# MarineRoboticsGroup/score

Measured on AMD Instinct MI355X. Metric: socp_iters_per_sec, higher is better.
Workload: dtype f64; 1 GPU; BASELINE configs[3]: manhattan RA-SLAM, 20 robots x 1000 poses, 4 beacons, SOCP relaxation, 1 trial(s)/GPU, ADMM loop alone (polish off) to eps 1e-07; n=146995, m=80979, nnz_P=946147, parallelism=independent x1

## Files before the change

score_amd/csrc/score_hip.hip:

```cpp
#include <hip/hip_runtime.h>
#include <sched.h>
#include <sys/prctl.h>
#include <time.h>
#include <hip/hip_ext.h>

#include <cstdio>
#include <cstring>
#include <malloc.h>
#include <mutex>
#include <string>
#include <memory>
#include <optional>
#include <vector>

#include "score_driver.hpp"
#include <future>
#include "score_assemble.hpp"
#include "score_gn_kernels.hpp"
#include "score_round.hpp"
#include "score_kernels.hpp"
#include "score_polish.hpp"
#include "score_polish_device.hpp"
#include "score_setup_device.hpp"
#include "score_prec_wave.hpp"
// ... 1840 lines not shown
            std::memset(h_rep, 0, total * sizeof(double));
            double* d_rep = nullptr;
            HIP_CHECK(hipHostGetDevicePointer((void**)&d_rep, h_rep, 0));
            rep.view(d_rep, total);
            rep_dres_off = n_pres;
            size_t o = 0;
            pres_part.view(d_rep + o, n_pres); h_pres = h_rep + o; o += n_pres;
            dres_part.view(d_rep + o, n_dres); h_dres = h_rep + o; o += n_dres;
            q_fpart.view(d_rep + o, n_fpart); h_newton = h_rep + o; o += n_fpart;
            q_gd.view(d_rep + o, n_gd); h_gd = h_rep + o; o += n_gd;
            h_meas = h_rep + o; d_meas = d_rep + o; o += n_meas;
            h_gate = (int32_t*)(h_rep + o); d_gate_host = (int32_t*)(d_rep + o); o += n_int;
            h_gate_live = (int32_t*)(h_rep + o); d_gate_live = (int32_t*)(d_rep + o); o += n_int;
            h_seq = (unsigned long long*)(h_rep + o); d_seq = (unsigned long long*)(d_rep + o);
            q_pcgdone.alloc(2 * (size_t)h.count);
            q_pcgdone.zero(stream);
            q_gate_used.view(q_pcgdone.d + h.count, h.count);
            ctl.alloc(2 * (size_t)h.count + (3 * (size_t)h.count + 1) / 2);
            q_step.view(ctl.d, h.count);
            q_gate_tol2.view(ctl.d + h.count, h.count);
            q_skip.view((int32_t*)(ctl.d + 2 * (size_t)h.count), h.count);
            q_reref.view((int32_t*)(ctl.d + 2 * (size_t)h.count) + h.count, h.count);
            q_fskip.view((int32_t*)(ctl.d + 2 * (size_t)h.count) + 2 * (size_t)h.count, h.count);
        }
        reset();
        pt.mark("reset");
        HIP_CHECK(sync_stream(stream));
        setup_tmp.release_all();
        for (auto& pb : setup_pinned) block_cache().give(pb.first, pb.second, st.device, true);
        setup_pinned.clear();
        pt.mark("staged uploads: drain");
    }

    void derive_rho_data(bool upload_penalties) {
        const HostSystem& h = *H;
        if (upload_penalties) {
            double* v = (double*)next_ring_slot(h.count * sizeof(double));
            for (int p = 0; p < h.count; ++p) v[p] = h.rho[p];
            fetch_words((int32_t*)rho.d, (const char*)v, 2 * h.count);
        }
        hipLaunchKernelGGL(k_kval, dim3(K.nblocks), dim3(kThreads), 0, stream, K.dev(), (const double*)K0d.d, (const double*)K1d.d,
                           (const double*)rho.d, K.val.d, (const int32_t*)nullptr);
        if (Kb.on) {
            const int64_t nnz = (int64_t)h.K.col.size();
            hipLaunchKernelGGL(k_band_pack, dim3((unsigned)((nnz + kThreads - 1) / kThreads)), dim3(kThreads), 0, stream, (const int32_t*)Kb.dst.d,
                               (const double*)K.val.d, Kb.V.d, nnz);
        }
        if (!h.factor_work.empty()) {
            FactorArgs fa{};
            fa.work = factor_work.d; fa.chains = chains.d; fa.levels = levels.d; fa.Hval = K.val.d;
            fa.pos_diag = kposd.d; fa.pos_sub = kposs.d; fa.fac = fac.d; fa.work_mat = q_work.d; fa.skip = nullptr;
            fa.diag_pos = kdiagpos.d; fa.dinv = dinv.d;
            launch_factor(fa, (int)h.factor_work.size(), false);
        }
        HIP_CHECK(hipGetLastError());
    }
    void join_init(const HostSystem& h) {
        n_join_items = (int)h.join_items.size(); n_join_chains = (int)h.join_chains.size(); n_join_seps = (int)h.join_sep_col.size();
        if (!n_join_items) return;
        for (const JoinChain& jc : h.join_chains)
            if (jc.n_seg - 1 > kJoinMaxSeps) throw std::runtime_error("internal: a segmented chain with more separators than the join kernel holds (build_system keeps such chains whole)");
        std::optional<UploadBatch> ub_join;
        ub_join.emplace();
        join_jc.upload(h.join_chains); join_items.upload(h.join_items);
        join_sep_col.upload(h.join_sep_col); join_sep_diag.upload(h.join_sep_diag);
        std::vector<int32_t> pc(2 * (size_t)n_join_seps), pp(2 * (size_t)n_join_seps);
// ... 613 lines not shown

    void launch_kp(const double* pdir, unsigned long long* ts = nullptr, int slot = -1) {
        SpmvArgs a = spmv_args(K, pdir);
        a.p = pdir; a.tstamp = ts;
        launch_spmv<MODE_KP>(K, a, slot);
    }
    void launch_kpb(const double* p_old, double* p_new, const double* rz_new, const double* rz_old,
                    unsigned long long* ts = nullptr, int slot = -1) {
        SpmvArgs a = spmv_args(K, p_old);
        a.tstamp = ts;
        a.p = p_old; a.z = z.d; a.p_out = p_new; a.rz_new = rz_new; a.rz_old = rz_old;
        launch_spmv<MODE_KPB>(K, a, slot);
    }

    void set_cg_iters(int k) {
        cg_iters = std::max(1, k);
        if (graph_exec) { (void)hipGraphExecDestroy(graph_exec); graph_exec = nullptr; }
    }

    void cg_reduction(std::vector<double>& out) {
        const HostSystem& h = *H;
        out.assign(h.count, 0.0);
        if (n_prec == 0) return;
        const double* a = h_meas;
        const double* b2 = h_meas + n_prec;
        for (int pi = 0; pi < h.count; ++pi) {
            double s0 = 0, s1 = 0;
            for (int i = active_part_ptr[pi]; i < active_part_ptr[pi + 1]; ++i) { s0 += a[i]; s1 += b2[i]; }
            out[pi] = s0 > 0 ? std::sqrt(std::max(0.0, s1) / s0) : 0.0;
        }
    }

    size_t ts_stride = 0;
    void enqueue_iteration(bool measure, bool first, unsigned long long* ts = nullptr) {
        auto slot = [&](int k) -> unsigned long long* { return ts ? ts + ts_stride * k : nullptr; };
        {
            SpmvArgs ra = spmv_args(G1, xtu.d);
            ra.tstamp = slot(0);
            ra.apply_update = first ? 0 : 1;
            ra.pfin = last_p;
            launch_spmv<MODE_RHS>(G1, ra, 0);
        }
        PrecArgs pa{};
        pa.work = prec_work.d; pa.chains = chains.d; pa.levels = levels.d; pa.rec = prec_rec.d; pa.fac = fac.d;
        pa.node_col = node_col.d; pa.diag_cols = diag_cols.d; pa.dinv = dinv.d; pa.done = done.d;
        pa.prec_part_ptr = prec_part_ptr.d; pa.kblk_part_ptr = kblk_part_ptr.d; pa.uni = uni_for(kblocks());
        pa.r = r.d; pa.r_in = r.d; pa.z = z.d; pa.p = p.d; pa.w = w.d; pa.xt = xtu.d; pa.kx = kx.d;
        pa.pw_part = pw_part.d;
        double* rz_cur = measure ? rz_meas0.d : rz_part0.d;
        double* p_cur = p.d;
        double* p_oth = p2.d;
        pa.p = p_cur; pa.rz_in = nullptr; pa.rz_out = rz_cur;
        pa.tstamp = slot(1);
        launch_prec<PREC_INIT>(pa, 1);
        launch_kp(p_cur, slot(2), 2);
        for (int j = 2; j <= cg_iters; ++j) {
            double* rz_nxt = (rz_cur == rz_part0.d) ? rz_part1.d : rz_part0.d;
            pa.p = p_cur; pa.rz_in = rz_cur; pa.rz_out = rz_nxt;
            pa.tstamp = (j == 2) ? slot(3) : nullptr;
            launch_prec<PREC_STEP>(pa, (j == 2) ? 3 : -1);
            launch_kpb(p_cur, p_oth, rz_nxt, rz_cur, (j == 2) ? slot(4) : nullptr, (j == 2) ? 4 : -1);
            std::swap(p_cur, p_oth);
            rz_cur = rz_nxt;
        }
        dbg_p = p_cur;
        ConeArgs ca = cone_args(xtu.d);
        if (measure) {
            pa.tstamp = nullptr;
            pa.p = p_cur; pa.rz_in = rz_cur; pa.rz_out = rz_meas1.d;
            launch_prec<PREC_STEP>(pa);
            VecArgs va{};
            va.first_row = vb_first.d; va.end_row = vb_end.d; va.blk_prob = vb_prob.d; va.done = done.d;
            va.prec_part_ptr = prec_part_ptr.d; va.kblk_part_ptr = kblk_part_ptr.d;
            va.pw_part = pw_part.d; va.p = p_cur; va.w = w.d; va.kx = kx.d; va.xt = xtu.d; va.x = xy.d;
            va.alpha_relax = st.alpha; va.rz_old = rz_cur; va.apply_alpha = 0;
            hipLaunchKernelGGL(k_xupdate, dim3(n_vblocks), dim3(kThreads), 0, stream, va);
        } else {
            ca.apply_alpha = 1; ca.pfin = p_cur; ca.rz_in = rz_cur;
            last_rz = rz_cur;
            last_p = p_cur;
        }
        ca.tstamp = slot(5);
        if (n_cone_blocks) {
            unsigned cgrid = (unsigned)n_cone_blocks;
            if (n_cone_blocks >= 16) { ca.xcd_chunk = (n_cone_blocks + 7) / 8; ca.n_blocks = n_cone_blocks; cgrid = 8u * (unsigned)ca.xcd_chunk; }
            launch_on_stream(k_cone, dim3(cgrid), dim3(kThreads), 0, 5, ca);
            ca.xcd_chunk = 0;
        }
        if (n_large_cones) {
            ca.tstamp = nullptr;
            hipLaunchKernelGGL(k_cone_wave, dim3((unsigned)((n_large_cones + 3) / 4)), dim3(kThreads), 0, stream, ca,
                               (const int2*)cone_large.d, n_large_cones);
        }
    }

    void time_iteration(int warmup, int iters, double* us, int with_events) {
        if (cg_iters != 2) throw std::runtime_error("score_time_iteration: needs cg_iters == 2");
        iters = std::max(1, iters);
        int khz = 0;
        HIP_CHECK(hipDeviceGetAttribute(&khz, hipDeviceAttributeWallClockRate, st.device));
        if (khz <= 0) throw std::runtime_error("score_time_iteration: no wall clock rate");
        for (int k = 0; k < 12; ++k) us[k] = 0.0;
        const int maxb = std::max(std::max(G1.nblocks, kblocks()) + 8, std::max(n_prec + n_help, n_cone_blocks + 8));
        ts_stride = (size_t)2 * maxb;
        const size_t per_iter = 6 * ts_stride, nslot = per_iter * iters;
        {
            std::vector<unsigned long long> hts(nslot);
            for (size_t i = 0; i < nslot; i += 2) { hts[i] = ~0ull; hts[i + 1] = 0ull; }
            DevBuf<unsigned long long> dts;
            dts.alloc(nslot);
            HIP_CHECK(hipMemcpyAsync(dts.d, hts.data(), nslot * sizeof(unsigned long long), hipMemcpyHostToDevice, stream));
            HIP_CHECK(sync_stream(stream));
            for (int i = 0; i < warmup; ++i) enqueue_iteration(false, i == 0);
            for (int i = 0; i < iters; ++i) enqueue_iteration(false, warmup == 0 && i == 0, dts.d + per_iter * i);
            HIP_CHECK(hipMemcpyAsync(hts.data(), dts.d, nslot * sizeof(unsigned long long), hipMemcpyDeviceToHost, stream));
            HIP_CHECK(sync_stream(stream));
            HIP_CHECK(hipGetLastError());
            for (int i = 0; i < iters; ++i)
                for (int k = 0; k < 6; ++k) {
                    const unsigned long long* p = &hts[per_iter * i + ts_stride * k];
                    unsigned long long t0 = ~0ull, t1 = 0ull;
                    for (int b = 0; b < maxb; ++b) { t0 = std::min(t0, p[2 * b]); t1 = std::max(t1, p[2 * b + 1]); }
                    if (t1 > t0) us[k] += (double)(t1 - t0) * 1e3 / (double)khz / iters;
                }
            if (trace_on("stamps")) {
                const unsigned long long* base = &hts[per_iter * (size_t)(iters - 1)];
                unsigned long long t00 = ~0ull;
                for (size_t j = 0; j < per_iter; j += 2) t00 = std::min(t00, base[j]);
                for (int k = 0; k < 6; ++k)
                    for (int b = 0; b < maxb; ++b) {
                        const unsigned long long a0 = base[ts_stride * k + 2 * (size_t)b], a1 = base[ts_stride * k + 2 * (size_t)b + 1];
                        if (a0 == ~0ull || a1 == 0ull) continue;
                        std::printf("STAMP %d %d %.3f %.3f\n", k, b, (double)(a0 - t00) * 1e3 / (double)khz, (double)(a1 - t00) * 1e3 / (double)khz);
                    }
            }
        }
        if (!with_events) return;
        std::vector<hipEvent_t> evs((size_t)12 * iters, nullptr);
        struct EvFree {
            std::vector<hipEvent_t>& v;
            ~EvFree() { for (hipEvent_t e : v) if (e) (void)hipEventDestroy(e); }
        } ev_free{evs};
        for (auto& e : evs) HIP_CHECK(hipEventCreate(&e));
        for (int i = 0; i < warmup; ++i) enqueue_iteration(false, false);
        for (int i = 0; i < iters; ++i) {
            tev = evs.data() + (size_t)12 * i;
            enqueue_iteration(false, false);
// ... 158 lines not shown
                               (const double*)Dd.d, (const double*)Ed.d, ob, n, m);
            try {
                copy_out({{x, {ob, (size_t)n}}, {y, {ob + n, (size_t)m}}, {s_out, {ob + n + m, (size_t)m}}});
            } catch (...) {
                block_cache().give(ob, got, st.device, false);
                throw;
            }
            block_cache().give(ob, got, st.device, false);
            return;
        }
        std::vector<double> hx((size_t)(n + m)), hs((size_t)m);
        copy_out({{hx.data(), {xy.d, hx.size()}}, {m ? hs.data() : nullptr, {s.d, hs.size()}}});
        if (x) for (int64_t i = 0; i < n; ++i) x[i] = hx[i] * h.D[i];
        if (y) for (int64_t i = 0; i < m; ++i) y[i] = hx[n + i] * h.E[i];
        if (s_out) for (int64_t i = 0; i < m; ++i) s_out[i] = hs[i] / h.E[i];
    }

    int64_t get_vec(const char* name, double* out, int64_t len) {
        const HostSystem& h = *H;
        const double* src = nullptr;
        int64_t sz = 0;
        bool host = false;
        std::string nm(name);
        if (nm == "xt") { src = xtu.d; sz = h.n_tot; }
        else if (nm == "u") { src = xtu.d + h.n_tot; sz = h.m_tot; }
        else if (nm == "x") { src = xy.d; sz = h.n_tot; }
        else if (nm == "y") { src = xy.d + h.n_tot; sz = h.m_tot; }
        else if (nm == "s") { src = s.d; sz = h.m_tot; }
        else if (nm == "r") { src = r.d; sz = h.n_tot; }
        else if (nm == "z") { src = z.d; sz = h.n_tot; }
        else if (nm == "p") { src = dbg_p ? dbg_p : ((cg_iters % 2 == 1) ? p.d : p2.d); sz = h.n_tot; }
        else if (nm == "w") { src = w.d; sz = h.n_tot; }
        else if (nm == "kx") { src = kx.d; sz = h.n_tot; }
        else if (nm == "D" && h.device_setup) { src = Dd.d; sz = h.n_tot; }
        else if (nm == "E" && h.device_setup) { src = Ed.d; sz = h.m_tot; }
        else if (nm == "D") { src = h.D.data(); sz = h.n_tot; host = true; }
        else if (nm == "E") { src = h.E.data(); sz = h.m_tot; host = true; }
        else if (nm == "K0" || nm == "K1" || nm == "Aval" || nm == "G1val" || nm == "G2val" || nm == "qs" || nm == "bs" || nm == "invD" || nm == "invE") {
            const int64_t nk = (int64_t)h.K.col.size(), na = (int64_t)h.A.ptr[(size_t)h.m_tot];
            const int64_t n1 = h.device_setup ? g1_nnz : (int64_t)h.G1.col.size(), n2 = (int64_t)h.G2.ptr[(size_t)h.n_tot];
            if (nm == "K0") { src = K0d.d; sz = nk; } else if (nm == "K1") { src = K1d.d; sz = nk; }
            else if (nm == "Aval") { src = A_val.d; sz = na; } else if (nm == "G1val") { src = G1.val.d; sz = n1; }
            else if (nm == "G2val") { src = G2.val.d; sz = n2; } else if (nm == "qs") { src = q.d; sz = h.n_tot; }
            else if (nm == "bs") { src = b.d; sz = h.m_tot; } else if (nm == "invD") { src = invD.d; sz = h.n_tot; }
            else { src = invE.d; sz = h.m_tot; }
        }
        else if (nm == "Acol" || nm == "Aptr" || nm == "G1col" || nm == "G1ptr" || nm == "G2col" || nm == "G2ptr" || nm == "G2split" || nm == "Kcol_dev" || nm == "Kptr_dev") {
            const int64_t nk = (int64_t)h.K.col.size(), na = (int64_t)h.A.ptr[(size_t)h.m_tot];
            const int64_t n1 = h.device_setup ? g1_nnz : (int64_t)h.G1.col.size(), n2 = (int64_t)h.G2.ptr[(size_t)h.n_tot];
            const int32_t* isrc = nullptr;
            if (nm == "Acol") { isrc = A_col.d; sz = na; } else if (nm == "Aptr") { isrc = A_ptr.d; sz = h.m_tot + 1; }
            else if (nm == "G1col") { isrc = G1.col.d; sz = n1; } else if (nm == "G1ptr") { isrc = G1.ptr.d; sz = h.n_tot + 1; }
            else if (nm == "G2col") { isrc = G2.col.d; sz = n2; } else if (nm == "G2ptr") { isrc = G2.ptr.d; sz = h.n_tot + 1; }
            else if (nm == "G2split") { isrc = G2.split.d; sz = h.n_tot; } else if (nm == "Kcol_dev") { isrc = K.col.d; sz = nk; }
            else { isrc = K.ptr.d; sz = h.n_tot + 1; }
            if (out && len > 0) {
                std::vector<int32_t> tmp((size_t)std::min(len, sz));
                HIP_CHECK(sync_stream(stream));
                staged_d2h(tmp.data(), isrc, tmp.size() * sizeof(int32_t), stream);
                HIP_CHECK(sync_stream(stream));
                for (size_t i = 0; i < tmp.size(); ++i) out[i] = (double)tmp[i];
            }
            return sz;
        }
        else if (nm == "setup_scalars") {
            sz = 5 * (int64_t)h.count;
// ... 5 lines not shown
            return sz;
        }
        else if (nm == "device_setup") {
            if (out && len > 0) out[0] = h.device_setup ? 1.0 : 0.0;
            return 1;
        }
        else if (nm == "Kval") { src = K.val.d; sz = (int64_t)h.K.col.size(); }
        else if (nm == "rep") {
            const double v[3] = {(double)h.rep, (double)h.K.col.size(), (double)(h.device_setup ? (size_t)g1_nnz : h.G1.col.size())};
            if (out && len > 0) std::memcpy(out, v, sizeof(double) * (size_t)std::min<int64_t>(len, 3));
            return 3;
        }
        else if (nm == "links") {
            double v[6] = {(double)link_plan.pairs_total, (double)link_plan.pairs_used, (double)n_link_u, (double)n_link_items, (double)link_rounds, 0.0};
            if (n_link_probs && out) {
                std::vector<int32_t> stt((size_t)n_link_probs);
                HIP_CHECK(sync_stream(stream));
                for (int set = 0; set < 2; ++set) {
                    if (!link_set_on[set]) continue;
                    HIP_CHECK(hipMemcpy(stt.data(), link_status[set].d, sizeof(int32_t) * (size_t)n_link_probs, hipMemcpyDeviceToHost));
                    for (int32_t x : stt) v[5] += x;
                }
            }
            if (out && len > 0) std::memcpy(out, v, sizeof(double) * (size_t)std::min<int64_t>(len, 6));
            return 6;
        }
        else if (nm == "link_pairs") {
            const std::vector<int32_t>& pc = link_plan.pair_cols;
            const int64_t np_ = n_link_items ? (int64_t)pc.size() : 0;
            if (out) for (int64_t i = 0; i < np_ && i < len; ++i) out[i] = (double)pc[(size_t)i];
            return np_;
        }
        else if (nm == "fac") { src = fac.d; sz = (int64_t)h.fac_doubles; }
        else if (nm == "newton_probe_arm") {
            if (!Q.available) return -1;
            if (out && len > 0) {
                for (hipEvent_t e : np_ev) (void)hipEventDestroy(e);
                np_ev.assign((size_t)2 * kProbeCap, nullptr);
                for (auto& e : np_ev)
                    if (hipEventCreate(&e) != hipSuccess) return -2;
                np_slots.clear();
                np_armed = true;
                out[0] = 1.0;
            }
            return 1;
        }
        else if ((nm == "ag_device_check" || nm == "polish_build_check") && h.device_setup) return -1;
        else if (nm == "ag_device_check") {
            if (out && len >= 7) {
                auto down_i = [&](const int32_t* d, size_t cnt) {
                    std::vector<int32_t> v(cnt);
                    if (cnt) staged_d2h(v.data(), d, cnt * sizeof(int32_t), stream);
                    HIP_CHECK(sync_stream(stream));
                    return v;
                };
                auto down_d = [&](const double* d, size_t cnt) {
                    std::vector<double> v(cnt);
                    if (cnt) staged_d2h(v.data(), d, cnt * sizeof(double), stream);
                    HIP_CHECK(sync_stream(stream));
                    return v;
                };
                auto mism = [](const std::vector<int32_t>& x, const std::vector<int32_t>& y) {
                    double c = 0;
                    for (size_t i = 0; i < y.size(); ++i) c += x[i] != y[i];
                    return c;
                };
// ... 1911 lines not shown
```

score_amd/csrc/score_host.hpp:

```cpp
#pragma once

#include <algorithm>
#include <atomic>
#include <cmath>
#include <chrono>
#include <cstdint>
#include <cstdio>
#include <cstring>
#include <numeric>
#include <stdexcept>
#include <string>
#include <thread>
#include <condition_variable>
#include <functional>
#include <mutex>

#include <pthread.h>
#include <sched.h>
#include <sys/resource.h>
#include <vector>

#include "../../include/score_hip.h"

namespace score {
// ... 547 lines not shown
}

inline void chain_level_layout(int bs, int radix, int N0, std::vector<ChainLevelDesc>& levels, size_t& fac_size,
                               int& scratch_nodes) {
    const int b2 = bs * bs;
    int N = N0, vec_off = 0, lds_off = 0;
    size_t off = 0;
    levels.clear();
    for (int lvl = 0;; ++lvl) {
        ChainLevelDesc L{};
        L.N = N;
        L.vec_off = (lvl == 0) ? -1 : vec_off;
        if (lvl > 0) vec_off += N;
        const bool last = (N <= radix - 1);
        L.p = last ? 0 : radix;
        L.inv_p = last ? 0u : ((1u << 20) / (uint32_t)radix + 1u);
        L.lds_off = lds_off;
        lds_off += N * bs + (last ? 0 : N / radix) + 1;
        const int nsep = last ? 0 : N / radix;
        L.nsep = nsep;
        L.nruns = nsep + 1;
        L.P = last ? N : radix - 1;
        L.offR = (int64_t)off; off += (size_t)2 * b2 * L.P * L.nruns;
        L.offS = (int64_t)off; off += (size_t)2 * b2 * nsep;
        L.offB = (int64_t)off; off += (size_t)2 * b2 * N;
        levels.push_back(L);
        if (last) break;
        N = nsep;
    }
    fac_size = off;
    scratch_nodes = vec_off;
}

inline bool chain_lane_plan(std::vector<ChainLevelDesc>& lv, int lanes) {
    for (auto& L : lv) { L.lane0 = -1; L.pad_ = 0; }
    if (lv.size() < 2) return true;
    bool ok = lv[1].N <= lanes && lv[1].nruns <= lanes;
    lv[1].lane0 = 0;
    int next = (lv[1].nruns + 63) / 64 * 64;
    for (size_t l = 2; l < lv.size() && ok; ++l) {
        const int need = std::max(lv[l].N, lv[l].nruns);
        if (next + need > lanes) { ok = false; break; }
        lv[l].lane0 = next;
        next = (next + need + 63) / 64 * 64;
    }
    if (!ok) {
        for (auto& L : lv) L.lane0 = -1;
        return ok;
    }
    int mask = 0;
    for (int w = 0; w * 64 < lanes && w < 4; ++w) {
        const int w0 = 64 * w;
        if (lv[1].p != 0 && w0 < lv[1].N) mask |= 1 << w;
        for (size_t l = 1; l < lv.size(); ++l) {
            if (lv[l].lane0 < w0 + 64 && lv[l].lane0 + lv[l].nruns > w0) mask |= 1 << (4 + w);
            if (l >= 2 && lv[l].p != 0 && lv[l].lane0 < w0 + 64 && lv[l].lane0 + lv[l].N > w0) mask |= 1 << (8 + w);
        }
    }
    lv[0].pad_ = mask;
    return ok;
}
inline int deep_group_pad(int bs) { return ((2 * bs * bs + 3) & ~3) - 2 * bs * bs; }
inline int deep_padded_slot(int bs, int slot) {
    const int b2 = bs * bs, pad = deep_group_pad(bs);
    return slot < 2 * b2 ? slot : (slot < 10 * b2 ? slot + pad : slot + 2 * pad);
}
inline int deep_padded_slots(int bs) { return 12 * bs * bs + 2 * deep_group_pad(bs); }
inline void chain_deep_map(int bs, const std::vector<ChainLevelDesc>& lv, int64_t fac_base, int lanes, std::vector<int32_t>& map) {
    const int b2 = bs * bs, RMAX = 3;
    map.assign((size_t)12 * b2 * lanes, -1);
    auto put = [&](int slot, int dt, int64_t idx) { map[(size_t)slot * lanes + dt] = (int32_t)(idx - fac_base); };
    for (size_t l = 1; l < lv.size(); ++l) {
        const ChainLevelDesc& L = lv[l];
        const bool last = (L.p == 0);
        for (int j = 0; j < L.nruns; ++j) {
            const int lo = last ? 0 : j * L.p;
            const int hi = last ? L.N : std::min(j * L.p + L.p - 1, L.N);
            const int len = std::max(hi - lo, 1);
            for (int q = 0; q < RMAX; ++q)
                for (int slot = 0; slot < 2; ++slot)
                    for (int e = 0; e < b2; ++e)
                        put(2 * b2 + (slot * RMAX + q) * b2 + e, L.lane0 + j,
                            L.offR + ((int64_t)(slot * b2 + e) * L.P + std::min(q, len - 1)) * L.nruns + j);
        }
        for (int j = 0; j < L.nsep; ++j)
            for (int slot = 0; slot < 2; ++slot)
                for (int e = 0; e < b2; ++e) put(2 * b2 + (2 * RMAX + slot) * b2 + e, L.lane0 + j, L.offS + (int64_t)(slot * b2 + e) * L.nsep + j);
        if (!last)
            for (int i = 0; i < L.N; ++i)
                for (int e = 0; e < 2 * b2; ++e) put((l == 1 ? 0 : 10 * b2) + e, L.lane0 + i, L.offB + (int64_t)e * L.N + i);
    }
}
// ... 1126 lines not shown
```

score_amd/csrc/score_kernels.hpp:

```cpp
#pragma once

#include <type_traits>

#include <hip/hip_runtime.h>

#include "score_host.hpp"
#include "score_band.hpp"

namespace score {

#ifdef SCORE_NT_STORES
#define NTS(lhs, val) __builtin_nontemporal_store((val), &(lhs))
#else
#define NTS(lhs, val) ((lhs) = (val))
#endif
#if defined(SCORE_NT_STORES) || defined(SCORE_NT_PREC)
#define NTSP(lhs, val) __builtin_nontemporal_store((val), &(lhs))
#else
#define NTSP(lhs, val) ((lhs) = (val))
#endif

constexpr int kThreads = 256;
constexpr int kUnroll = kTileNnz / kThreads;
constexpr int kLongUnroll = 2;
// ... 62 lines not shown
}
template <int NW>
__device__ __forceinline__ double reduce_partials_n(const double* __restrict__ part, int lo, int hi, double* red) {
    double acc = 0.0;
    for (int i = lo + (int)threadIdx.x; i < hi; i += NW * 64) acc += part[i];
    return block_sum_n<NW>(acc, red);
}

struct CsrDev {
    const int32_t* ptr;
    const int32_t* col;
    const double* val;
    const int32_t* first_row;
    const int32_t* blk_prob;
    const int4* blk_meta;
    const int32_t* blk_rs;
    const int32_t* split;
    int nblocks;
    const int4* blk_long;
    double* long_part;
    unsigned long long* long_cnt;
    int long_spin;
};
constexpr unsigned long long kLongSentinel = 0x7ff8dead7ff8deadull;
constexpr unsigned kLongSentinel32 = 0x7ff8deadu;

struct KernelStamp {
    unsigned long long* ts;
    __device__ explicit KernelStamp(unsigned long long* p) : ts(p) {
        if (ts && threadIdx.x == 0) ts[2 * blockIdx.x] = (unsigned long long)wall_clock64();
    }
    __device__ ~KernelStamp() {
        if (ts && threadIdx.x == 0) ts[2 * blockIdx.x + 1] = (unsigned long long)wall_clock64();
    }
};

struct UniRanges {
    int on;
    int l0, l1;
    int k0, k1;
};

struct BandDev {
    const double* val;
    const int32_t* rem_col;
    const int32_t* rowseg;
    const int4* meta2;
    int32_t rem0;
    int32_t bs;
    int32_t offw[kBandMaxS / 2];
};

struct SpmvArgs {
    UniRanges uni;
    CsrDev M;
    BandDev B;
    const double* xin;
    const int32_t* done;
    int xcd_chunk;
    int n_tiles;
    int early_done;
    int rs_in;
    const double* x;
    const double* q;
    const double* kx;
    double* r;
// ... 716 lines not shown
struct alignas(16) PrecRecord {
    PrecWork wk;
    ChainDesc ch;
    int32_t pad_;
    ChainLevelDesc lv[kRecLevels];
};
static_assert(sizeof(PrecRecord) == 512, "PrecRecord is read as 32 int4");

struct PrecArgs {
    const PrecWork* work;
    const PrecRecord* rec;
    const ChainDesc* chains;
    const ChainLevelDesc* levels;
    const double* fac;
    const float* fac32;
    const float* deep;
    const int32_t* node_col;
    const int32_t* diag_cols;
    const double* dinv;
    const int32_t* done;
    const int32_t* prec_part_ptr;
    const int32_t* kblk_part_ptr;
    UniRanges uni;
    double* r;
    double* z;
    double* p;
    const double* w;
    double* xt;
    double* kx;
    const double* rz_in;
    const double* pw_part;
    double* rz_out;
    unsigned long long* tstamp;
    int debug_skip;
    int n_vec;
    long long vec_stride;
    int split_update;
    const double* r_in;
    int xt_zero;
    int early_done;
    int32_t* gate_init;
    int32_t* gate_flag;
    const double* gate_tol2;
    double* gate_ref;
    int32_t* gate_used;
    int gate_first;
    int32_t* gate_host;
    int32_t gate_epoch, gate_count;
};

enum { PREC_INIT = 0, PREC_STEP = 1 };



__device__ __forceinline__ bool pcg_gate(const PrecArgs& a, int prob, double rz, double ref_loaded) {
    if (!a.gate_flag) return false;
    const bool lead = (threadIdx.x == 0) && ((int)blockIdx.x == a.prec_part_ptr[prob]);
    if (a.gate_first) {
        if (!(rz > 0.0)) {
            if (lead) { a.gate_flag[prob] = 1; if (a.gate_host) a.gate_host[prob] = a.gate_epoch; }
            return true;
        }
        if (lead) {
            a.gate_ref[prob] = rz * a.gate_tol2[prob]; a.gate_used[prob] = 1;
            if (a.gate_host) a.gate_host[a.gate_count + prob] = (a.gate_epoch << 12) | 1;
        }
// ... 478 lines not shown
    double local = 0.0;
    if (wk.kind == 2) {
        if (dn || dn_late) return;
        if (MODE == PREC_INIT) return;
        const double gref = (a.gate_flag && !a.gate_first) ? a.gate_ref[prob] : 0.0;
        const int e_end = wk.index + wk.count;
        int idx[kPrecChunk];
        double pv[kPrecChunk], wv[kPrecChunk], xv[kPrecChunk], kv[kPrecChunk];
#pragma unroll
        for (int u = 0; u < kPrecChunk; ++u) {
            idx[u] = min(wk.index + t + u * kPrecThreads, e_end - 1);
            pv[u] = a.p[idx[u]]; wv[u] = a.w[idx[u]]; xv[u] = a.xt_zero ? 0.0 : a.xt[idx[u]]; kv[u] = a.kx[idx[u]];
        }
        block_sum2_n<kPrecWaves>(acc_rz, acc_pw, red);
        const double alpha = acc_pw > 0.0 ? acc_rz / acc_pw : 0.0;
        if (a.gate_flag && (a.gate_first ? !(acc_rz > 0.0) : !(acc_rz > gref))) return;
#pragma unroll
        for (int u = 0; u < kPrecChunk; ++u) {
            if (wk.index + t + u * kPrecThreads < e_end) {
                NTSP(a.xt[idx[u]], xv[u] + alpha * pv[u]);
                NTSP(a.kx[idx[u]], kv[u] + alpha * wv[u]);
            }
        }
        return;
    }
    if (wk.kind == 1) {
        if (dn || dn_late) return;
        bool stop;
        local = prec_jacobi_item<MODE>(a, wk, acc_rz, acc_pw, red, stop);
        if (stop) return;
    } else {
        const double gref = (MODE == PREC_STEP && a.gate_flag && !a.gate_first) ? a.gate_ref[prob] : 0.0;
        const ChainDesc ch = srec.ch;
        const FT* __restrict__ fac = sizeof(FT) == 4 ? (const FT*)(const void*)a.fac32 : (const FT*)(const void*)a.fac;
        const int N = ch.N;
        const int NB = N * BS;
        const int nl = ch.n_levels;
        const int stride = ch.col_stride, col0 = ch.col0;
        auto colof = [&](int node) -> int { return col0 + node * stride; };
        double* vb = lds + 16;
        double* v0 = vb;
        const ChainLevelDesc L0 = sLv[0];
        const ChainLevelDesc Lz = sLv[nl - 1];
        LT* lfac = reinterpret_cast<LT*>(vb + Lz.lds_off + Lz.N * BS + 1);
        auto pad = [](const ChainLevelDesc& L, int i) -> int { return (int)(((uint32_t)i * L.inv_p) >> 20); };
        auto nodep = [&](const ChainLevelDesc& L, int i) -> double* { return vb + L.lds_off + i * BS + pad(L, i); };
        int64_t deep_base = 0;
        int deep_cnt = 0;
        if (nl >= 2) {
            deep_base = sLv[1].offR;
            deep_cnt = (int)(Lz.offB + (int64_t)2 * B2 * Lz.N - deep_base);
        }
        double* xch = REGDEEP ? vb + Lz.lds_off + Lz.N * BS + 1 : reinterpret_cast<double*>(lfac + ((deep_cnt + 1) & ~1));
        int cols[CH];
        double rv[CH], wv[CH];
#pragma unroll
        for (int u = 0; u < CH; ++u) {
            const int idx = min(t + u * kPrecThreads, NB - 1);
            const int node = idx / BS;
            cols[u] = colof(node) + (idx - node * BS);
        }
        constexpr bool kLateW = (BS >= 4);
#pragma unroll
        for (int u = 0; u < CH; ++u) {
            rv[u] = a.r_in[cols[u]];
            if (MODE == PREC_STEP && !kLateW) wv[u] = a.w[cols[u]];
        }
        FT Gr[NG];
        const bool l0_last = (L0.p == 0);
        if (t < kPreRunLanes) {
            if ((t & ~63) < L0.nruns && !(a.debug_skip & 1)) {
                const int j = min(t, L0.nruns - 1);
                const int lo = l0_last ? 0 : j * L0.p;
                const int hi = l0_last ? L0.N : min(j * L0.p + L0.p - 1, L0.N);
                const int len = max(hi - lo, 1);
                const size_t eP = (size_t)L0.P * L0.nruns;
                const FT* __restrict__ R = fac + L0.offR;
#pragma unroll
                for (int q = 0; q < RMAX; ++q) {
// ... 68 lines not shown
            for (int u = 0; u < CH; ++u) wv[u] = a.w[cols[u]];
        }
#pragma unroll
        for (int u = 0; u < CH; ++u) {
            const int idx = t + u * kPrecThreads;
            if (idx < NB) {
                double r_ = rv[u];
                if (MODE == PREC_STEP) {
                    r_ -= alpha * wv[u];
                    NTSP(a.r[cols[u]], r_);
                }
                v0[idx + pad(L0, idx / BS)] = r_;
                rv[u] = r_;
            }
        }
        if (t >= kPreRunLanes && !REGDEEP) {
            if (deep_cnt > 0 && !(a.debug_skip & 2)) {
                const int lane = t - kPreRunLanes;
#pragma unroll
                for (int k0 = 0; k0 < NG; k0 += 8) {
                    if (k0 * kStageLanes < deep_cnt) {
#pragma unroll
                        for (int k = k0; k < k0 + 8; ++k) {
                            const int idx = lane + k * kStageLanes;
                            if (idx < deep_cnt) lfac[idx] = (LT)Gr[k];
                        }
                    }
                }
            }
        }
        LT G[NG];
#pragma unroll
        for (int k = 0; k < NG; ++k) G[k] = (LT)Gr[k];
        lds_barrier();
        auto run_solve0 = [&](double (&y)[RMAX][BS], int len) {
#pragma unroll
            for (int q = 1; q < RMAX; ++q) {
#pragma unroll
                for (int c = 0; c < BS; ++c) {
                    double s_ = y[q][c];
#pragma unroll
                    for (int k = 0; k < BS; ++k) s_ -= G[oRun + q * B2 + c * BS + k] * y[q - 1][k];
                    y[q][c] = s_;
                }
            }
#pragma unroll
            for (int q = RMAX - 1; q >= 0; --q) {
                double tmp[BS];
#pragma unroll
                for (int c = 0; c < BS; ++c) {
                    double s_ = 0.0;
#pragma unroll
                    for (int k = 0; k < BS; ++k) s_ += G[oRun + (RMAX + q) * B2 + c * BS + k] * y[q][k];
                    tmp[c] = s_;
                }
                if (q + 1 < RMAX) {
                    const bool has_next = (q + 1 < len);
#pragma unroll
                    for (int c = 0; c < BS; ++c) {
                        double s_ = 0.0;
#pragma unroll
                        for (int k = 0; k < BS; ++k) s_ += G[oRun + (q + 1) * B2 + k * BS + c] * y[q + 1][k];
                        tmp[c] = has_next ? tmp[c] - s_ : tmp[c];
                    }
                }
#pragma unroll
                for (int c = 0; c < BS; ++c) y[q][c] = tmp[c];
            }
        };
        const bool dbg_nophase = (a.debug_skip & 4) != 0;
        if (t < L0.nruns && !dbg_nophase) {
            const int j = t;
            const int lo = l0_last ? 0 : j * L0.p;
            const int hi = l0_last ? L0.N : min(j * L0.p + L0.p - 1, L0.N);
            const int len = hi - lo;
            const int jpad = l0_last ? 0 : j;
            if (len > 0) {
                double y[RMAX][BS];
#pragma unroll
                for (int q = 0; q < RMAX; ++q) {
                    const double* src = v0 + (lo + min(q, len - 1)) * BS + jpad;
#pragma unroll
                    for (int c = 0; c < BS; ++c) y[q][c] = src[c];
                }
                run_solve0(y, len);
#pragma unroll
                for (int q = 0; q < RMAX; ++q) {
                    if (q < len) {
                        double* dst = v0 + (lo + q) * BS + jpad;
#pragma unroll
                        for (int c = 0; c < BS; ++c) dst[c] = y[q][c];
                    }
                }
            }
        }
        lds_barrier();
        if (nl >= 2 && !dbg_nophase) {
            const ChainLevelDesc L1 = sLv[1];
            if (t < L0.nsep) {
                const int s = t * L0.p + L0.p - 1;
                const bool has_r = (s + 1 < L0.N);
                const double* pv_ = v0 + s * BS + t;
                const double* pm = v0 + (s - 1) * BS + t;
                const double* pp = has_r ? v0 + (s + 1) * BS + t + 1 : pv_;
                double v[BS], ym[BS], yp[BS];
#pragma unroll
                for (int c = 0; c < BS; ++c) { v[c] = pv_[c]; ym[c] = pm[c]; yp[c] = pp[c]; }
#pragma unroll
                for (int c = 0; c < BS; ++c) {
                    double acc = v[c];
#pragma unroll
                    for (int k = 0; k < BS; ++k) acc -= G[oCl + c * BS + k] * ym[k] + G[oCr + c * BS + k] * yp[k];
                    nodep(L1, t)[c] = acc;
                }
            }
            lds_barrier();
        }
        constexpr int kHalf = CH / 2;
        double pv[kHalf], wq[kHalf], xv[kHalf], kv[kHalf];
        auto upd_load = [&](auto half) {
            constexpr int u0 = decltype(half)::value * kHalf;
#pragma unroll
            for (int u = 0; u < kHalf; ++u) {
                pv[u] = a.p[cols[u0 + u]]; wq[u] = a.w[cols[u0 + u]]; xv[u] = a.xt_zero ? 0.0 : a.xt[cols[u0 + u]]; kv[u] = a.kx[cols[u0 + u]];
            }
        };
        auto upd_store = [&](auto half) {
            constexpr int u0 = decltype(half)::value * kHalf;
#pragma unroll
            for (int u = 0; u < kHalf; ++u) {
                if (t + (u0 + u) * kPrecThreads < NB) {
                    NTSP(a.xt[cols[u0 + u]], xv[u] + alpha * pv[u]);
                    NTSP(a.kx[cols[u0 + u]], kv[u] + alpha * wq[u]);
                }
            }
        };
        using H0 = std::integral_constant<int, 0>;
        using H1 = std::integral_constant<int, 1>;
        constexpr bool kLateUpdate = (BS >= 4);
        const bool own_update = (MODE == PREC_STEP) && !a.split_update;
        if (own_update && !kLateUpdate) upd_load(H0());
        const int dt = t - kPreRunLanes;
        for (int l = 1; l < nl && !dbg_nophase; ++l) {
            const ChainLevelDesc L = sLv[l];
            const bool last = (L.p == 0);
            const int dl = REGDEEP ? dt - L.lane0 : dt;
            if (dt >= 0 && dl >= 0 && dl < L.nruns) {
                const int j = dl;
                const int lo = last ? 0 : j * L.p;
                const int hi = last ? L.N : min(j * L.p + L.p - 1, L.N);
                const int len = hi - lo;
                if (len > 0) {
                    if (!REGDEEP) {
                        const int eP = L.P * L.nruns;
                        const LT* R = lfac + (L.offR - deep_base);
#pragma unroll
                        for (int q = 0; q < RMAX; ++q) {
                            const LT* Rq = R + min(q, len - 1) * L.nruns + j;
#pragma unroll
                            for (int e = 0; e < B2; ++e) {
                                G[q * B2 + e] = Rq[e * eP];
                                G[(RMAX + q) * B2 + e] = Rq[(B2 + e) * eP];
                            }
                        }
                    }
                    double* vr = vb + L.lds_off + lo * BS + (last ? 0 : j);
                    double y[RMAX][BS];
#pragma unroll
                    for (int q = 0; q < RMAX; ++q)
#pragma unroll
                        for (int c = 0; c < BS; ++c) y[q][c] = vr[min(q, len - 1) * BS + c];
                    run_solve0(y, len);
#pragma unroll
                    for (int q = 0; q < RMAX; ++q) {
                        if (q < len) {
#pragma unroll
                            for (int c = 0; c < BS; ++c) vr[q * BS + c] = y[q][c];
                        }
                    }
                }
            }
            lds_barrier();
            if (last) break;
            const ChainLevelDesc Ln = sLv[l + 1];
            if (dt >= 0 && dl >= 0 && dl < L.nsep) {
                const int js = dl;
                if (!REGDEEP) {
                    const LT* S = lfac + (L.offS - deep_base);
#pragma unroll
                    for (int e = 0; e < B2; ++e) {
                        G[oCl + e] = S[e * L.nsep + js];
                        G[oCr + e] = S[(B2 + e) * L.nsep + js];
                    }
                }
                const int s = js * L.p + L.p - 1;
                const bool has_r = (s + 1 < L.N);
                const double* pv_ = vb + L.lds_off + s * BS + js;
                const double* pm = vb + L.lds_off + (s - 1) * BS + js;
                const double* pp = has_r ? vb + L.lds_off + (s + 1) * BS + js + 1 : pv_;
                double v[BS], ym[BS], yp[BS];
#pragma unroll
                for (int c = 0; c < BS; ++c) { v[c] = pv_[c]; ym[c] = pm[c]; yp[c] = pp[c]; }
                double* dst = nodep(Ln, js);
#pragma unroll
                for (int c = 0; c < BS; ++c) {
                    double acc = v[c];
#pragma unroll
                    for (int k = 0; k < BS; ++k) acc -= G[oCl + c * BS + k] * ym[k] + G[oCr + c * BS + k] * yp[k];
                    dst[c] = acc;
                }
            }
            lds_barrier();
        }
        for (int l = nl - 2; l >= 1 && !dbg_nophase; --l) {
            const ChainLevelDesc Lb = sLv[l];
            const ChainLevelDesc Ln = sLv[l + 1];
            const int db = REGDEEP ? dt - Lb.lane0 : dt;
            if (dt >= 0 && db >= 0 && db < Lb.N) {
                const int i = db;
                LT Vw[2 * B2];
                if (REGDEEP) {
#pragma unroll
                    for (int e = 0; e < 2 * B2; ++e) Vw[e] = (l == 1) ? G[e] : G[oBk2 + e];
                } else {
                    const LT* Bk = lfac + (Lb.offB - deep_base);
#pragma unroll
                    for (int e = 0; e < 2 * B2; ++e) Vw[e] = Bk[e * Lb.N + i];
                }
                const int nsep = Lb.nsep;
                const int j = pad(Lb, i);
                const bool is_sep = (i - j * Lb.p == Lb.p - 1) && (j < nsep);
                const int jl = max(j - 1, 0), jr = min(j, max(nsep - 1, 0));
                double* pvx = vb + Lb.lds_off + i * BS + j;
                const double* pul = nodep(Ln, jl);
                const double* pur = nodep(Ln, jr);
                double v[BS], ul[BS], ur[BS];
#pragma unroll
                for (int c = 0; c < BS; ++c) { v[c] = pvx[c]; ul[c] = pul[c]; ur[c] = pur[c]; }
#pragma unroll
                for (int c = 0; c < BS; ++c) {
                    double acc = v[c];
#pragma unroll
                    for (int k = 0; k < BS; ++k) acc -= Vw[c * BS + k] * ul[k] + Vw[B2 + c * BS + k] * ur[k];
                    pvx[c] = is_sep ? ur[c] : acc;
                }
            }
            lds_barrier();
        }
        if (own_update && !kLateUpdate) { upd_store(H0()); upd_load(H1()); }
        if (nl >= 2 && !dbg_nophase) {
            const ChainLevelDesc L1 = sLv[1];
            const int nsep = L0.nsep;
            double c_last[BS];
#pragma unroll
            for (int c = 0; c < BS; ++c) c_last[c] = 0.0;
            if (t < nsep) {
                const int s = t * L0.p + L0.p - 1;
                double xs[BS];
#pragma unroll
                for (int c = 0; c < BS; ++c) xs[c] = nodep(L1, t)[c];
#pragma unroll
                for (int c = 0; c < BS; ++c) {
                    double sl = 0.0, sr = 0.0;
#pragma unroll
                    for (int k = 0; k < BS; ++k) { sl += G[oCl + k * BS + c] * xs[k]; sr += G[oCr + k * BS + c] * xs[k]; }
                    c_last[c] = sl;
                    xch[(size_t)(t + 1) * BS + c] = sr;
                    v0[s * BS + t + c] = xs[c];
                }
            }
            lds_barrier();
            if (t < L0.nruns) {
                const int lo = t * L0.p;
                const int hi = min(t * L0.p + L0.p - 1, L0.N);
                const int len = hi - lo;
                if (len > 0) {
                    double y[RMAX][BS];
#pragma unroll
                    for (int q = 0; q < RMAX; ++q)
#pragma unroll
                        for (int c = 0; c < BS; ++c) {
                            double v = (q == len - 1) ? c_last[c] : 0.0;
                            if (q == 0 && t >= 1) v += xch[(size_t)t * BS + c];
                            y[q][c] = v;
                        }
                    run_solve0(y, len);
#pragma unroll
                    for (int q = 0; q < RMAX; ++q) {
                        if (q < len) {
                            double* dst = v0 + (lo + q) * BS + t;
#pragma unroll
                            for (int c = 0; c < BS; ++c) dst[c] -= y[q][c];
                        }
                    }
                }
            }
            lds_barrier();
        }
        if (own_update && !kLateUpdate) upd_store(H1());
        if (own_update && kLateUpdate) { upd_load(H0()); upd_store(H0()); upd_load(H1()); upd_store(H1()); }
#pragma unroll
        for (int u = 0; u < CH; ++u) {
            const int idx = t + u * kPrecThreads;
            if (idx < NB) {
                const double zz = v0[idx + pad(L0, idx / BS)];
                NTSP(a.z[cols[u]], zz);
                if (MODE == PREC_INIT) NTSP(a.p[cols[u]], zz);
                local += rv[u] * zz;
            }
        }
    }
    const double tot = block_sum_n<kPrecWaves>(local, red);
    if (t == 0) a.rz_out[blockIdx.x] = tot;
}

struct VecArgs {
    const int32_t* first_row;
    const int32_t* end_row;
    const int32_t* blk_prob;
    const int32_t* done;
    const int32_t* prec_part_ptr;
    const int32_t* kblk_part_ptr;
    const double* rz_old;
    const double* pw_part;
    const double* p;
    const double* w;
    double* kx;
    double* xt;
    double* x;
    double alpha_relax;
    int apply_alpha;
};

__global__ __launch_bounds__(kThreads) void k_xupdate(VecArgs a) {
    __shared__ double red[8];
    const int b = blockIdx.x;
    const int prob = a.blk_prob[b];
    if (a.done[prob]) return;
    double alpha = 0.0;
    if (a.apply_alpha) {
        const double rz = reduce_partials(a.rz_old, a.prec_part_ptr[prob], a.prec_part_ptr[prob + 1], red);
        const double pw = reduce_partials(a.pw_part, a.kblk_part_ptr[prob], a.kblk_part_ptr[prob + 1], red);
        alpha = pw > 0.0 ? rz / pw : 0.0;
// ... 417 lines not shown
```

Before: 17610 iters/s.

## Pack deep-chain lane plan into shared waves and use wave syncs where possible

Changes the chain lane planner to pack successive tree levels contiguously within a 64-lane wave instead of aligning each level to a wave boundary. It then records a bitmask of barrier points whose producer and consumer lanes lie in the same wave, and the preconditioner kernel replaces those block-wide LDS barriers with cheaper wave syncs. It also adds optional compile-time phase timestamps and a debug hook that re-plans lanes at runtime. The risk is correctness if the hand-off mask is wrong and wave-level sync is insufficient.

```diff
diff --git a/score_amd/csrc/score_hip.hip b/score_amd/csrc/score_hip.hip
--- a/score_amd/csrc/score_hip.hip
+++ b/score_amd/csrc/score_hip.hip
@@ -1896,6 +1896,46 @@
         pt.mark("staged uploads: drain");
     }
 
+    void use_lane_plan(bool packed) {
+        const HostSystem& h = *H;
+        if (!prec_reg) return;
+        constexpr int kLanes = kPrecThreads - kPreRunLanes;
+        std::vector<ChainLevelDesc> lv = h.levels, lvH = h.levelsH;
+        std::vector<int32_t> map = h.deep_map;
+        auto replan = [&](const std::vector<ChainDesc>& cs, std::vector<ChainLevelDesc>& ls) {
+            for (const ChainDesc& ch : cs) {
+                if (ch.deep_map_off < 0) continue;
+                std::vector<ChainLevelDesc> one(ls.begin() + ch.level_begin, ls.begin() + ch.level_begin + ch.n_levels);
+                if (!chain_lane_plan(one, kLanes, packed)) throw std::runtime_error("use_lane_plan: a chain does not fit");
+                std::copy(one.begin(), one.end(), ls.begin() + ch.level_begin);
+                std::vector<int32_t> mp;
+                chain_deep_map(h.bs, one, one[0].offR, kLanes, mp);
+                std::copy(mp.begin(), mp.end(), map.begin() + ch.deep_map_off);
+            }
+        };
+        replan(h.chains, lv);
+        replan(h.chainsH, lvH);
+        HIP_CHECK(sync_stream(stream));
+        auto put = [&](auto* d, const auto& v) { HIP_CHECK(hipMemcpy(d, v.data(), v.size() * sizeof(v[0]), hipMemcpyHostToDevice)); };
+        put(levels.d, lv);
+        if (levelsH.d != levels.d) put(levelsH.d, lvH);
+        put(deep_map.d, map);
+        auto patch = [&](DevBuf<PrecRecord>& rb, const std::vector<ChainDesc>& cs, const std::vector<ChainLevelDesc>& ls) {
+            std::vector<PrecRecord> rec(rb.n);
+            HIP_CHECK(hipMemcpy(rec.data(), rb.d, rec.size() * sizeof(PrecRecord), hipMemcpyDeviceToHost));
+            for (PrecRecord& r : rec) {
+                if (r.wk.kind != 0) continue;
+                const ChainDesc& ch = cs[(size_t)r.wk.index];
+                for (int l = 0; l < std::min<int>(ch.n_levels, kRecLevels); ++l) r.lv[l] = ls[(size_t)ch.level_begin + l];
+            }
+            put(rb.d, rec);
+        };
+        patch(prec_rec, h.chains, lv);
+        if (prec_recH.d != prec_rec.d) patch(prec_recH, h.chainsH, lvH);
+        derive_rho_data(false);
+        HIP_CHECK(sync_stream(stream));
+    }
+
     void derive_rho_data(bool upload_penalties) {
         const HostSystem& h = *H;
         if (upload_penalties) {
@@ -2575,6 +2615,7 @@
     }
 
     size_t ts_stride = 0;
+    unsigned long long* phase_ts = nullptr;
     void enqueue_iteration(bool measure, bool first, unsigned long long* ts = nullptr) {
         auto slot = [&](int k) -> unsigned long long* { return ts ? ts + ts_stride * k : nullptr; };
         {
@@ -2595,13 +2636,18 @@
         double* p_oth = p2.d;
         pa.p = p_cur; pa.rz_in = nullptr; pa.rz_out = rz_cur;
         pa.tstamp = slot(1);
+        const size_t phase_stride = (size_t)(n_prec + n_help) * kPhaseStamps * 8;
+        pa.pstamp = phase_ts;
         launch_prec<PREC_INIT>(pa, 1);
+        pa.pstamp = nullptr;
         launch_kp(p_cur, slot(2), 2);
         for (int j = 2; j <= cg_iters; ++j) {
             double* rz_nxt = (rz_cur == rz_part0.d) ? rz_part1.d : rz_part0.d;
             pa.p = p_cur; pa.rz_in = rz_cur; pa.rz_out = rz_nxt;
             pa.tstamp = (j == 2) ? slot(3) : nullptr;
+            pa.pstamp = (j == 2 && phase_ts) ? phase_ts + phase_stride : nullptr;
             launch_prec<PREC_STEP>(pa, (j == 2) ? 3 : -1);
+            pa.pstamp = nullptr;
             launch_kpb(p_cur, p_oth, rz_nxt, rz_cur, (j == 2) ? slot(4) : nullptr, (j == 2) ? 4 : -1);
             std::swap(p_cur, p_oth);
             rz_cur = rz_nxt;
@@ -2653,9 +2699,38 @@
             DevBuf<unsigned long long> dts;
             dts.alloc(nslot);
             HIP_CHECK(hipMemcpyAsync(dts.d, hts.data(), nslot * sizeof(unsigned long long), hipMemcpyHostToDevice, stream));
+#ifdef SCORE_PHASE_STAMPS
+            const bool phases = trace_on("stamps");
+#else
+            const bool phases = false;
+#endif
+            const size_t ph_launch = (size_t)(n_prec + n_help) * kPhaseStamps * 8, ph_iter = 2 * ph_launch;
+            DevBuf<unsigned long long> dph;
+            if (phases) {
+                dph.alloc(ph_iter * iters);
+                HIP_CHECK(hipMemsetAsync(dph.d, 0, ph_iter * iters * sizeof(unsigned long long), stream));
+            }
             HIP_CHECK(sync_stream(stream));
             for (int i = 0; i < warmup; ++i) enqueue_iteration(false, i == 0);
-            for (int i = 0; i < iters; ++i) enqueue_iteration(false, warmup == 0 && i == 0, dts.d + per_iter * i);
+            for (int i = 0; i < iters; ++i) {
+                phase_ts = phases ? dph.d + ph_iter * i : nullptr;
+                enqueue_iteration(false, warmup == 0 && i == 0, dts.d + per_iter * i);
+            }
+            phase_ts = nullptr;
+            if (phases) {
+                std::vector<unsigned long long> hph(ph_iter * iters);
+                HIP_CHECK(hipMemcpyAsync(hph.data(), dph.d, hph.size() * sizeof(unsigned long long), hipMemcpyDeviceToHost, stream));
+                HIP_CHECK(sync_stream(stream));
+                std::printf("PHASECLK %d\n", khz);
+                for (int i = 0; i < iters; ++i)
+                    for (int k = 0; k < 2; ++k)
+                        for (int b = 0; b < n_prec + n_help; ++b)
+                            for (int w = 0; w < 8; ++w)
+                                for (int q = 0; q < kPhaseStamps; ++q) {
+                                    const unsigned long long v = hph[ph_iter * i + ph_launch * k + ((size_t)b * kPhaseStamps + q) * 8 + w];
+                                    if (v) std::printf("PHASE %d %d %d %d %d %llu\n", i, k, b, w, q, v);
+                                }
+            }
             HIP_CHECK(hipMemcpyAsync(hts.data(), dts.d, nslot * sizeof(unsigned long long), hipMemcpyDeviceToHost, stream));
             HIP_CHECK(sync_stream(stream));
             HIP_CHECK(hipGetLastError());
@@ -2880,6 +2955,7 @@
         else if (nm == "p") { src = dbg_p ? dbg_p : ((cg_iters % 2 == 1) ? p.d : p2.d); sz = h.n_tot; }
         else if (nm == "w") { src = w.d; sz = h.n_tot; }
         else if (nm == "kx") { src = kx.d; sz = h.n_tot; }
+        else if (nm == "rz_part") { src = rz_part1.d; sz = n_prec; }
         else if (nm == "D" && h.device_setup) { src = Dd.d; sz = h.n_tot; }
         else if (nm == "E" && h.device_setup) { src = Ed.d; sz = h.m_tot; }
         else if (nm == "D") { src = h.D.data(); sz = h.n_tot; host = true; }
@@ -2951,6 +3027,13 @@
             return np_;
         }
         else if (nm == "fac") { src = fac.d; sz = (int64_t)h.fac_doubles; }
+        else if (nm == "lane_plan_old" || nm == "lane_plan_packed") {
+            if (out && len > 0) {
+                use_lane_plan(nm == "lane_plan_packed");
+                out[0] = prec_reg ? 1.0 : 0.0;
+            }
+            return 1;
+        }
         else if (nm == "newton_probe_arm") {
             if (!Q.available) return -1;
             if (out && len > 0) {
diff --git a/score_amd/csrc/score_host.hpp b/score_amd/csrc/score_host.hpp
--- a/score_amd/csrc/score_host.hpp
+++ b/score_amd/csrc/score_host.hpp
@@ -603,17 +603,18 @@
     scratch_nodes = vec_off;
 }
 
-inline bool chain_lane_plan(std::vector<ChainLevelDesc>& lv, int lanes) {
+inline bool chain_lane_plan(std::vector<ChainLevelDesc>& lv, int lanes, bool packed = true) {
     for (auto& L : lv) { L.lane0 = -1; L.pad_ = 0; }
     if (lv.size() < 2) return true;
     bool ok = lv[1].N <= lanes && lv[1].nruns <= lanes;
     lv[1].lane0 = 0;
-    int next = (lv[1].nruns + 63) / 64 * 64;
+    int next = lv[1].nruns;
     for (size_t l = 2; l < lv.size() && ok; ++l) {
         const int need = std::max(lv[l].N, lv[l].nruns);
+        if (!packed || next % 64 + need > 64) next = (next + 63) / 64 * 64;
         if (next + need > lanes) { ok = false; break; }
         lv[l].lane0 = next;
-        next = (next + need + 63) / 64 * 64;
+        next += need;
     }
     if (!ok) {
         for (auto& L : lv) L.lane0 = -1;
@@ -629,6 +630,23 @@
         }
     }
     lv[0].pad_ = mask;
+    if (packed) {
+        auto wave = [](int lo, int n) { return lo / 64 == (lo + n - 1) / 64 ? lo / 64 : -1; };
+        auto one = [&](int lo0, int n0, int lo1, int n1) { return wave(lo0, n0) >= 0 && wave(lo0, n0) == wave(lo1, n1); };
+        int hand = 0;
+        const int nl = (int)lv.size();
+        for (int l = 1; l < nl && l < 8; ++l) {
+            const ChainLevelDesc& L = lv[l];
+            if (L.p != 0) {
+                if (one(L.lane0, L.nruns, L.lane0, L.nsep)) hand |= 1 << l;
+                if (one(L.lane0, L.nsep, lv[l + 1].lane0, lv[l + 1].nruns)) hand |= 1 << (8 + l);
+                if (l >= 2 && one(L.lane0, L.N, lv[l - 1].lane0, lv[l - 1].N)) hand |= 1 << (16 + l);
+            } else if (l >= 2 && one(L.lane0, L.nruns, lv[l - 1].lane0, lv[l - 1].N)) {
+                hand |= 1 << l;
+            }
+        }
+        lv[1].pad_ = hand;
+    }
     return ok;
 }
 inline int deep_group_pad(int bs) { return ((2 * bs * bs + 3) & ~3) - 2 * bs * bs; }
diff --git a/score_amd/csrc/score_kernels.hpp b/score_amd/csrc/score_kernels.hpp
--- a/score_amd/csrc/score_kernels.hpp
+++ b/score_amd/csrc/score_kernels.hpp
@@ -118,6 +118,44 @@
     }
     __device__ ~KernelStamp() {
         if (ts && threadIdx.x == 0) ts[2 * blockIdx.x + 1] = (unsigned long long)wall_clock64();
+    }
+};
+
+constexpr int kPhaseStamps = 48;
+struct PhaseStamp {
+    template <class A>
+    __device__ static __forceinline__ void put(const A& a, int k, unsigned long long v) {
+#ifdef SCORE_PHASE_STAMPS
+        if (a.pstamp && (threadIdx.x & 63) == 0) a.pstamp[((size_t)blockIdx.x * kPhaseStamps + k) * 8 + (threadIdx.x >> 6)] = v;
+#else
+        (void)a; (void)k; (void)v;
+#endif
+    }
+    template <class A>
+    __device__ static __forceinline__ void at(const A& a, int k) {
+#ifdef SCORE_PHASE_STAMPS
+        put(a, k, (unsigned long long)__builtin_amdgcn_s_memtime());
+#else
+        (void)a; (void)k;
+#endif
+    }
+    template <class A>
+    __device__ static __forceinline__ void entry(const A& a) {
+#ifdef SCORE_PHASE_STAMPS
+        put(a, 46, (unsigned long long)wall_clock64());
+        at(a, 44);
+#else
+        (void)a;
+#endif
+    }
+    template <class A>
+    __device__ static __forceinline__ void exit(const A& a) {
+#ifdef SCORE_PHASE_STAMPS
+        at(a, 45);
+        put(a, 47, (unsigned long long)wall_clock64());
+#else
+        (void)a;
+#endif
     }
 };
 
@@ -900,6 +938,7 @@
     const double* pw_part;
     double* rz_out;
     unsigned long long* tstamp;
+    unsigned long long* pstamp;
     int debug_skip;
     int n_vec;
     long long vec_stride;
@@ -1444,6 +1483,7 @@
     } else {
         const double gref = (MODE == PREC_STEP && a.gate_flag && !a.gate_first) ? a.gate_ref[prob] : 0.0;
         const ChainDesc ch = srec.ch;
+        PhaseStamp::entry(a);
         const FT* __restrict__ fac = sizeof(FT) == 4 ? (const FT*)(const void*)a.fac32 : (const FT*)(const void*)a.fac;
         const int N = ch.N;
         const int NB = N * BS;
@@ -1457,6 +1497,13 @@
         LT* lfac = reinterpret_cast<LT*>(vb + Lz.lds_off + Lz.N * BS + 1);
         auto pad = [](const ChainLevelDesc& L, int i) -> int { return (int)(((uint32_t)i * L.inv_p) >> 20); };
         auto nodep = [&](const ChainLevelDesc& L, int i) -> double* { return vb + L.lds_off + i * BS + pad(L, i); };
+        const int hand = (REGDEEP && nl >= 2) ? __builtin_amdgcn_readfirstlane(sLv[1].pad_) : 0;
+        auto sync_at = [&](int b, int bit) {
+            PhaseStamp::at(a, 2 * b);
+            if (bit >= 0 && ((hand >> bit) & 1)) wave_sync();
+            else lds_barrier();
+            PhaseStamp::at(a, 2 * b + 1);
+        };
         int64_t deep_base = 0;
         int deep_cnt = 0;
         if (nl >= 2) {
@@ -1591,7 +1638,7 @@
         LT G[NG];
 #pragma unroll
         for (int k = 0; k < NG; ++k) G[k] = (LT)Gr[k];
-        lds_barrier();
+        sync_at(0, -1);
         auto run_solve0 = [&](double (&y)[RMAX][BS], int len) {
 #pragma unroll
             for (int q = 1; q < RMAX; ++q) {
@@ -1653,7 +1700,7 @@
                 }
             }
         }
-        lds_barrier();
+        sync_at(1, -1);
         if (nl >= 2 && !dbg_nophase) {
             const ChainLevelDesc L1 = sLv[1];
             if (t < L0.nsep) {
@@ -1673,7 +1720,7 @@
                     nodep(L1, t)[c] = acc;
                 }
             }
-            lds_barrier();
+            sync_at(2, -1);
         }
         constexpr int kHalf = CH / 2;
         double pv[kHalf], wq[kHalf], xv[kHalf], kv[kHalf];
@@ -1739,7 +1786,7 @@
                     }
                 }
             }
-            lds_barrier();
+            sync_at(2 * l + 1, l);
             if (last) break;
             const ChainLevelDesc Ln = sLv[l + 1];
             if (dt >= 0 && dl >= 0 && dl < L.nsep) {
@@ -1769,7 +1816,7 @@
                     dst[c] = acc;
                 }
             }
-            lds_barrier();
+            sync_at(2 * l + 2, 8 + l);
         }
         for (int l = nl - 2; l >= 1 && !dbg_nophase; --l) {
             const ChainLevelDesc Lb = sLv[l];
@@ -1804,7 +1851,7 @@
                     pvx[c] = is_sep ? ur[c] : acc;
                 }
             }
-            lds_barrier();
+            sync_at(14 + l, 16 + l);
         }
         if (own_update && !kLateUpdate) { upd_store(H0()); upd_load(H1()); }
         if (nl >= 2 && !dbg_nophase) {
@@ -1828,7 +1875,7 @@
                     v0[s * BS + t + c] = xs[c];
                 }
             }
-            lds_barrier();
+            sync_at(20, -1);
             if (t < L0.nruns) {
                 const int lo = t * L0.p;
                 const int hi = min(t * L0.p + L0.p - 1, L0.N);
@@ -1854,7 +1901,7 @@
                     }
                 }
             }
-            lds_barrier();
+            sync_at(21, -1);
         }
         if (own_update && !kLateUpdate) upd_store(H1());
         if (own_update && kLateUpdate) { upd_load(H0()); upd_store(H0()); upd_load(H1()); upd_store(H1()); }
@@ -1868,6 +1915,7 @@
                 local += rv[u] * zz;
             }
         }
+        PhaseStamp::exit(a);
     }
     const double tot = block_sum_n<kPrecWaves>(local, red);
     if (t == 0) a.rz_out[blockIdx.x] = tot;
```

Result: no change. 17540 iters/s, median of 3 (-0.4%).
